# icbi-lab/infercnvpy

Hardware: AMD Instinct MI355X
Metric: cells/sec through tl.infercnv (window=100), input resident in HBM (higher is better)
Workload: dtype f64

## Files before the change

infercnvpy_amd/csrc/icv_api.hip:

```cpp
#include "../../include/infercnv_hip.h"

#include <hip/hip_runtime.h>

#include <algorithm>
#include <atomic>
#include <cmath>
#include <cstdio>
#include <cstdlib>
#include <cstring>
#include <mutex>
#include <new>
#include <string>
#include <system_error>
#include <thread>
#if defined(__x86_64__)
#include <immintrin.h>
#endif
#include <memory>
#include <vector>

#include <rocprim/device/device_radix_sort.hpp>
#include <rocprim/device/device_reduce_by_key.hpp>
#include <rocprim/device/device_scan.hpp>

// ... 1176 lines not shown
        partial_off = 0;
        start_off = up(partial_off + (size_t)n_slabs * nc * 8);
        slab_rec_off = up(start_off + (size_t)n_slabs * nc * 8);
        rec_off = up(slab_rec_off + (size_t)n_slabs * nc * 4);
        count_off = up(rec_off + (size_t)n_blocks * nc * 4);
        stash_off = up(count_off + 256);
        const size_t want = (size_t)n_blocks * nc / 32 + 4096;
        stash_cap = (unsigned)(want < 0x7ffffff0u ? want : 0x7ffffff0u);
        bytes = up(stash_off + (size_t)stash_cap * icv::kBkRows * 4);
    }
};
int blocks_check(const icv_matrix* m, const void* ws) {
    if (!m || !ws) return fail(ICV_ERR_INVALID, "null matrix or workspace");
    if (m->format != ICV_DENSE || m->dtype != ICV_F32)
        return fail(ICV_ERR_UNSUPPORTED, "the block form of the chain takes dense float32 matrices (others: icv_colchain)");
    if (m->n_rows < 0 || m->n_cols < 1 || m->ld < m->n_cols) return fail(ICV_ERR_INVALID, "bad matrix");
    return ICV_OK;
}
}

int icv_colchain_blocks_workspace(int64_t n_rows, int32_t n_cols, int64_t* bytes) {
    if (!bytes || n_rows < 0 || n_cols < 1) return fail(ICV_ERR_INVALID, "bad colchain_blocks_workspace arguments");
    *bytes = (int64_t)BlocksLayout(n_rows, n_cols).bytes;
    return ICV_OK;
}

int icv_colchain_blocks_sums(const icv_matrix* m, void* workspace, double* total, void* stream) {
    int rc = blocks_check(m, workspace);
    if (rc) return rc;
    if (!total) return fail(ICV_ERR_INVALID, "total is required");
    hipStream_t st = static_cast<hipStream_t>(stream);
    const BlocksLayout L(m->n_rows, m->n_cols);
    double* partial = reinterpret_cast<double*>(static_cast<char*>(workspace) + L.partial_off);
    HIP_TRY(hipMemsetAsync(total, 0, (size_t)m->n_cols * sizeof(double), st));
    if (m->n_rows == 0) return ICV_OK;
    dim3 grid((m->n_cols + 255) / 256, (unsigned)L.n_slabs);
    hipLaunchKernelGGL(icv::k_colsum_dense<float>, grid, dim3(256), 0, st, (const float*)m->values, m->n_rows, m->ld,
                       m->n_cols, (const int32_t*)nullptr, 0, icv::kBkSlab, partial);
    hipLaunchKernelGGL(icv::k_colsum_finish, dim3((m->n_cols + 63) / 64), dim3(1024), 0, st, partial, (int)L.n_slabs,
                       m->n_cols, total);
    HIP_TRY(hipGetLastError());
    return ICV_OK;
}

int icv_colchain_blocks_records(const icv_matrix* m, void* workspace, const double* est_start, void* stream) {
    int rc = blocks_check(m, workspace);
    if (rc) return rc;
    if (m->n_rows == 0) return ICV_OK;
    hipStream_t st = static_cast<hipStream_t>(stream);
    const BlocksLayout L(m->n_rows, m->n_cols);
    char* w = static_cast<char*>(workspace);
    const double* partial = reinterpret_cast<const double*>(w + L.partial_off);
    double* slab_start = reinterpret_cast<double*>(w + L.start_off);
    HIP_TRY(hipMemsetAsync(w + L.count_off, 0, 256, st));
    hipLaunchKernelGGL(icv::k_blocks_prefix, dim3((m->n_cols + 255) / 256), dim3(256), 0, st, partial, (int)L.n_slabs,
                       m->n_cols, est_start, slab_start);
    dim3 grid((m->n_cols + 255) / 256, (unsigned)L.n_slabs);
    hipLaunchKernelGGL(icv::k_chain_records, grid, dim3(256), 0, st, (const float*)m->values, m->n_rows, m->ld, m->n_cols,
                       slab_start, reinterpret_cast<uint32_t*>(w + L.rec_off), reinterpret_cast<uint32_t*>(w + L.slab_rec_off),
                       reinterpret_cast<float*>(w + L.stash_off), reinterpret_cast<unsigned*>(w + L.count_off), L.stash_cap);
    HIP_TRY(hipGetLastError());
    return ICV_OK;
}

int icv_colchain_blocks_scan(const icv_matrix* m, void* workspace, float* acc, int32_t col0, int32_t col1,
                             uint64_t* d_replayed, void* stream) {
    int rc = blocks_check(m, workspace);
    if (rc) return rc;
    if (!acc || col0 < 0 || col1 > m->n_cols || col0 > col1) return fail(ICV_ERR_INVALID, "bad colchain_blocks_scan arguments");
    if (m->n_rows == 0 || col1 == col0) return ICV_OK;
    hipStream_t st = static_cast<hipStream_t>(stream);
    const BlocksLayout L(m->n_rows, m->n_cols);
    char* w = static_cast<char*>(workspace);
    const int nc = col1 - col0;
    int64_t grid = ((int64_t)nc + 3) / 4;
    const int64_t cap = (int64_t)current_cu_count() * 8;
    if (grid > cap) grid = cap;
    hipLaunchKernelGGL(icv::k_chain_scan, dim3((unsigned)grid), dim3(256), 0, st,
                       (const float*)m->values + col0, m->n_rows, m->ld, nc, (int64_t)m->n_cols,
                       reinterpret_cast<const uint32_t*>(w + L.rec_off) + col0,
                       reinterpret_cast<const uint32_t*>(w + L.slab_rec_off) + col0,
                       reinterpret_cast<const float*>(w + L.stash_off), acc + col0,
                       reinterpret_cast<unsigned long long*>(d_replayed));
    HIP_TRY(hipGetLastError());
    return ICV_OK;
}

int icv_colchain(const icv_matrix* m, const int32_t* rows, int64_t n_sel, double scale, void* acc, void* stream) {
    if (!m || !acc) return fail(ICV_ERR_INVALID, "bad colchain arguments");
    if (m->dtype != ICV_F32 && m->dtype != ICV_F64) return fail(ICV_ERR_INVALID, "dtype must be ICV_F32 or ICV_F64");
    if (!rows) n_sel = m->n_rows;
    if (n_sel < 0 || n_sel > m->n_rows) return fail(ICV_ERR_INVALID, "icv_colchain: n_sel out of range");
    if (n_sel == 0 || m->n_cols == 0) return ICV_OK;
    hipStream_t st = static_cast<hipStream_t>(stream);
    if (m->format == ICV_CSR)
        return m->dtype == ICV_F32 ? colchain_csr<float>(m, rows, n_sel, scale, (float*)acc, st)
                                   : colchain_csr<double>(m, rows, n_sel, scale, (double*)acc, st);
    if (m->format != ICV_DENSE) return fail(ICV_ERR_INVALID, "format must be dense or csr");
    return m->dtype == ICV_F32 ? colchain_dense<float>(m, rows, n_sel, (float*)acc, st)
                               : colchain_dense<double>(m, rows, n_sel, (double*)acc, st);
}

int icv_colchain_mean(const void* acc, int32_t dtype, int32_t n_cols, int64_t count, void* mean, void* stream) {
    if (!acc || !mean || count < 1 || n_cols < 0) return fail(ICV_ERR_INVALID, "bad colchain_mean arguments");
    hipStream_t st = static_cast<hipStream_t>(stream);
    if (n_cols == 0) return ICV_OK;
    if (dtype == ICV_F32)
        hipLaunchKernelGGL(k_chain_mean<float>, dim3((n_cols + 255) / 256), dim3(256), 0, st, (const float*)acc, n_cols,
                           (float)count, (float*)mean);
    else if (dtype == ICV_F64)
        hipLaunchKernelGGL(k_chain_mean<double>, dim3((n_cols + 255) / 256), dim3(256), 0, st, (const double*)acc,
                           n_cols, (double)count, (double*)mean);
    else
        return fail(ICV_ERR_INVALID, "dtype must be ICV_F32 or ICV_F64");
    HIP_TRY(hipGetLastError());
    return ICV_OK;
}

int icv_colmean_csc(const void* values, int32_t dtype, const int64_t* colptr, const int32_t* row_idx, int32_t n_cols,
                    const int32_t* row_group, int32_t group, double scale, void* mean, void* stream) {
    if (!values || !colptr || !row_idx || !mean || n_cols < 0) return fail(ICV_ERR_INVALID, "bad colmean_csc arguments");
    hipStream_t st = static_cast<hipStream_t>(stream);
    if (n_cols == 0) return ICV_OK;
    if (dtype == ICV_F32)
        hipLaunchKernelGGL(icv::k_colpair_csc<float>, dim3((n_cols + 63) / 64), dim3(64), 0, st, (const float*)values,
                           colptr, row_idx, n_cols, row_group, group, (float)scale, (float*)mean);
    else if (dtype == ICV_F64)
        hipLaunchKernelGGL(icv::k_colpair_csc<double>, dim3((n_cols + 63) / 64), dim3(64), 0, st, (const double*)values,
                           colptr, row_idx, n_cols, row_group, group, scale, (double*)mean);
    else
        return fail(ICV_ERR_INVALID, "dtype must be ICV_F32 or ICV_F64");
    HIP_TRY(hipGetLastError());
    return ICV_OK;
}

int icv_colsum_pairwise(const void* xt, int32_t dtype, int64_t n_rows, int32_t n_cols, int64_t ld, void* sums,
                        void* stream) {
    if (!xt || !sums || n_rows < 0 || n_cols < 0 || ld < n_rows) return fail(ICV_ERR_INVALID, "bad colsum_pairwise arguments");
    hipStream_t st = static_cast<hipStream_t>(stream);
    if (n_cols == 0) return ICV_OK;
    if (dtype == ICV_F32)
        hipLaunchKernelGGL(icv::k_colpair_dense<float>, dim3((n_cols + 63) / 64), dim3(64), 0, st, (const float*)xt,
                           n_rows, n_cols, ld, (float*)sums);
    else if (dtype == ICV_F64)
        hipLaunchKernelGGL(icv::k_colpair_dense<double>, dim3((n_cols + 63) / 64), dim3(64), 0, st, (const double*)xt,
                           n_rows, n_cols, ld, (double*)sums);
    else
        return fail(ICV_ERR_INVALID, "dtype must be ICV_F32 or ICV_F64");
    HIP_TRY(hipGetLastError());
    return ICV_OK;
}

int icv_infercnv_smooth(icv_plan_t pl, const icv_matrix* m, const void* ref_lo, const void* ref_hi,
                        double lfc_clip, int32_t flags, float* out, int64_t ldo, double* cell_median,
                        double* cell_stats, void* stream) {
    int rc = check_matrix(pl, m);
    if (rc) return rc;
    PLAN_BUSY_GUARD(pl);
    if (!cell_median || !cell_stats) return fail(ICV_ERR_INVALID, "cell_median and cell_stats are required");
    if ((rc = ensure_device(pl))) return rc;
    PLAN_ENTER(stream);
    icv::KParams K;
    const icv::Layout* lay;
    if ((rc = fill_params(pl, m, ref_lo, ref_hi, lfc_clip, flags, out, ldo, cell_median, cell_stats, K, lay)))
        return rc;
    return launch_smooth(pl, m, K, *lay, static_cast<hipStream_t>(stream));
}

int icv_chunk_thresholds(const double* cell_stats, int64_t n_rows, int64_t chunksize, int64_t row_phase,
                         int32_t n_windows, double dynamic_threshold, double* thr, void* stream) {
    if (!cell_stats || !thr || chunksize < 1 || row_phase < 0 || row_phase >= chunksize)
        return fail(ICV_ERR_INVALID, "bad chunk threshold arguments");
    if (n_rows < 1) return ICV_OK;
    const int64_t n_chunks = (n_rows + row_phase + chunksize - 1) / chunksize;
    hipLaunchKernelGGL(icv::k_chunk_thr, dim3((unsigned)n_chunks), dim3(256), 0, static_cast<hipStream_t>(stream),
                       cell_stats, n_rows, chunksize, row_phase, n_windows, dynamic_threshold, thr);
    HIP_TRY(hipGetLastError());
    return ICV_OK;
}

int icv_apply_threshold(icv_plan_t pl, const icv_matrix* m, const void* ref_lo, const void* ref_hi,
                        double lfc_clip, int32_t flags, float* out, int64_t ldo, const double* cell_median,
                        const double* thr, int64_t chunksize, int64_t row_phase, void* stream) {
    int rc = check_matrix(pl, m);
    if (rc) return rc;
    PLAN_BUSY_GUARD(pl);
    if (!cell_median || !thr || chunksize < 1) return fail(ICV_ERR_INVALID, "bad apply_threshold arguments");
    if ((rc = ensure_device(pl))) return rc;
    PLAN_ENTER(stream);
    icv::KParams K;
    const icv::Layout* lay;
    if ((rc = fill_params(pl, m, ref_lo, ref_hi, lfc_clip, flags, out, ldo, const_cast<double*>(cell_median),
                          nullptr, K, lay)))
        return rc;
    return launch_apply(m, K, thr, chunksize, row_phase, static_cast<hipStream_t>(stream));
}

}

namespace {
int run_steps(icv_plan_t pl, const icv_matrix* m, const void* ref_lo, const void* ref_hi, double lfc_clip,
              double dynamic_threshold, int64_t chunksize, int64_t row_phase, int32_t flags, float* out, int64_t ldo,
              double* cell_median, double* cell_stats, double* thr, icv_profile* prof, double* win_out, int64_t ldw,
              void* stream) {
    int rc;
    const bool do_thr = !std::isnan(dynamic_threshold);
    hipStream_t st = static_cast<hipStream_t>(stream);
    icv::KParams K;
    const icv::Layout* lay;
    if ((rc = fill_params(pl, m, ref_lo, ref_hi, lfc_clip, flags, out, ldo, cell_median, cell_stats, K, lay)))
        return rc;
    K.win_out = win_out;
    K.win_ld = ldw;
    bool chunk_mode = false;
    int64_t n_chunks = 1, cs_eff = m->n_rows > 0 ? m->n_rows : 1, ph_eff = 0;
    if (do_thr) {
        cs_eff = chunksize;
        ph_eff = row_phase;
        n_chunks = (m->n_rows + row_phase + chunksize - 1) / chunksize;
        if (n_chunks < 1) n_chunks = 1;
    }
    if (!cell_stats && m->n_rows > 0) {
        if (pl->hb_stats_cap < m->n_rows) {
            (void)hipFree(pl->d_hb_stats);
            pl->d_hb_stats = nullptr;
            pl->hb_stats_cap = 0;
            HIP_TRY(hipMalloc((void**)&pl->d_hb_stats, (size_t)m->n_rows * 2 * sizeof(double)));
            pl->hb_stats_cap = m->n_rows;
        }
        K.cell_stats = pl->d_hb_stats;
        const int64_t se_slots = ((int64_t)pl->n_cu * (icv::kLdsLimit / icv::kSeLds)) * icv::NWAVE;
        const int64_t x16_slots = (int64_t)pl->n_cu * icv::XWAVE;
        const int64_t n_part = se_slots > x16_slots ? se_slots : x16_slots;
        if ((x16_applies(pl, m, K, *lay) || stored_entries_kernel(pl, m, K, *lay)) &&
            n_chunks * n_part <= (int64_t)(64 << 20) / 16) {
            chunk_mode = true;
            if (pl->chunk_part_cap < n_chunks * n_part) {
                (void)hipFree(pl->d_chunk_part);
                pl->d_chunk_part = nullptr;
                pl->chunk_part_cap = 0;
                HIP_TRY(hipMalloc((void**)&pl->d_chunk_part, (size_t)(n_chunks * n_part) * 2 * sizeof(double)));
                pl->chunk_part_cap = n_chunks * n_part;
            }
            HIP_TRY(hipMemsetAsync(pl->d_chunk_part, 0, (size_t)(n_chunks * n_part) * 2 * sizeof(double), st));
            HIP_TRY(hipMemsetAsync(pl->d_hb_stats, 0, (size_t)m->n_rows * 2 * sizeof(double), st));
            K.chunk_part = pl->d_chunk_part;
            K.chunksize = cs_eff;
            K.row_phase = ph_eff;
        }
    }
    EventSet evs;
    hipEvent_t* ev = evs.ev;
    const bool deferred = !prof && pl->prof_deferred;
    const bool timed = prof || deferred;
    if (timed) {
        for (int i = 0; i < 4; ++i) HIP_TRY(hipEventCreate(&ev[i]));
        HIP_TRY(hipEventRecord(ev[0], st));
    }
    bool ev1_done = false;
    if ((rc = launch_smooth(pl, m, K, *lay, st, timed ? ev[1] : nullptr, &ev1_done))) return rc;
    if (timed && !ev1_done) HIP_TRY(hipEventRecord(ev[1], st));
    if (do_thr && chunk_mode) {
        int64_t n_slots;
        if (m->format == ICV_CSR) {
            n_slots = se_grid(pl, m->n_rows) * icv::NWAVE;
        } else {
            int64_t gx = pl->n_cu;
            if (gx > m->n_rows) gx = m->n_rows;
            n_slots = gx * icv::XWAVE;
        }
        hipLaunchKernelGGL(icv::k_chunk_thr_part, dim3((unsigned)n_chunks), dim3(256), 0, st, pl->d_chunk_part,
                           (int)n_slots, pl->d_hb_stats, m->n_rows, chunksize, row_phase, pl->p.W,
                           dynamic_threshold, thr);
        HIP_TRY(hipGetLastError());
    } else if (do_thr && m->n_rows > 0) {
        rc = icv_chunk_thresholds(K.cell_stats, m->n_rows, chunksize, row_phase, pl->p.W, dynamic_threshold, thr,
                                  stream);
        if (rc) return rc;
    }
    if (timed) HIP_TRY(hipEventRecord(ev[2], st));
    if (do_thr && !(flags & ICV_FLAG_NO_APPLY) && (rc = launch_apply(m, K, thr, chunksize, row_phase, st))) return rc;
    if (timed) HIP_TRY(hipEventRecord(ev[3], st));
    if (deferred) {
        for (int i = 0; i < 4; ++i) pl->prof_events.push_back(ev[i]);
        evs.keep = true;
    } else if (prof) {
        HIP_TRY(hipEventSynchronize(ev[3]));
        HIP_TRY(hipEventElapsedTime(&prof->smooth_ms, ev[0], ev[1]));
        HIP_TRY(hipEventElapsedTime(&prof->thresholds_ms, ev[1], ev[2]));
        HIP_TRY(hipEventElapsedTime(&prof->apply_ms, ev[2], ev[3]));
        HIP_TRY(hipEventElapsedTime(&prof->total_ms, ev[0], ev[3]));
    }
    return ICV_OK;
}

int gene_from_windows(icv_plan_t pl, const double* win, int64_t ldw, int64_t n, const double* thr, int64_t chunksize,
                      int64_t row_phase, double* gene_out, int64_t ldg, hipStream_t st) {
    const icv::Plan& p = pl->p;
    if (n < 1) return ICV_OK;
    const int W = p.W, n_cov = (int)p.cov_col.size(), R = (int)p.gv_run_j0.size();
    const bool pk_lds = icv::gv_lds_bytes(W, R, pl->gv_mult_bytes, true) * 2 <= (size_t)icv::kLdsLimit;
    const size_t lds = icv::gv_lds_bytes(W, R, pl->gv_mult_bytes, pk_lds);
    if (lds <= (size_t)icv::kLdsLimit && pl->gv_fused_ok && !knobs().no_gene_fused) {
        HIP_TRY(hipFuncSetAttribute(reinterpret_cast<const void*>(icv::k_gene_fused),
                                    hipFuncAttributeMaxDynamicSharedMemorySize, (int)lds));
        int per_cu = (int)((size_t)icv::kLdsLimit / lds);
        if (per_cu > 2048 / icv::kGvThreads) per_cu = 2048 / icv::kGvThreads;
        int64_t grid = (int64_t)pl->n_cu * per_cu;
        if (grid > n) grid = n;
        hipLaunchKernelGGL(icv::k_gene_fused, dim3((unsigned)grid), dim3(icv::kGvThreads), lds, st, win, ldw, n, W,
                           pl->d_gv_pk, pl->d_gv_mult, R, n_cov, pl->d_gv_col16, p.n_cols_all, thr,
                           chunksize > 0 ? chunksize : 1, row_phase, gene_out, ldg, pl->gv_mult_bytes, (int)pk_lds);
        HIP_TRY(hipGetLastError());
        return ICV_OK;
    }
    AsyncBuf b_gv, b_med;
    HIP_TRY(b_gv.alloc((size_t)n * (n_cov > 0 ? n_cov : 1) * sizeof(double), st));
    HIP_TRY(b_med.alloc((size_t)n * sizeof(double), st));
    double *gv = b_gv.as<double>(), *med = b_med.as<double>();
    {
        const int64_t total = n * ldg;
        hipLaunchKernelGGL(icv::k_fill_nan, dim3((unsigned)((total + 255) / 256)), dim3(256), 0, st, gene_out, total);
    }
    if (n_cov > 0) {
        for (int64_t r0 = 0; r0 < n; r0 += 32768) {
            const int64_t nr = (n - r0) < 32768 ? (n - r0) : 32768;
            dim3 grid((n_cov + 255) / 256, (unsigned)nr);
            hipLaunchKernelGGL(icv::k_gene_means, grid, dim3(256), 0, st, win + r0 * ldw, nr, (int)ldw, pl->d_cov_j0,
                               pl->d_cov_cnt, n_cov, gv + r0 * n_cov);
        }
        hipLaunchKernelGGL(icv::k_row_median, dim3((unsigned)n), dim3(256), 0, st, gv, n, n_cov, med);
        for (int64_t r0 = 0; r0 < n; r0 += 32768) {
            const int64_t nr = (n - r0) < 32768 ? (n - r0) : 32768;
            dim3 grid((n_cov + 255) / 256, (unsigned)nr);
            hipLaunchKernelGGL(icv::k_gene_finish, grid, dim3(256), 0, st, gv + r0 * n_cov, med + r0, thr,
                               chunksize > 0 ? chunksize : 1, row_phase + r0, pl->d_cov_col, n_cov, gene_out + r0 * ldg,
                               ldg);
        }
    }
    HIP_TRY(hipGetLastError());
    return ICV_OK;
}
}

extern "C" {

int icv_infercnv_run(icv_plan_t pl, const icv_matrix* m, const void* ref_lo, const void* ref_hi, double lfc_clip,
                     double dynamic_threshold, int64_t chunksize, int64_t row_phase, int32_t flags, float* out,
                     int64_t ldo, double* cell_median, double* cell_stats, double* thr, icv_profile* prof,
                     void* stream) {
    return icv_infercnv_run_windows(pl, m, ref_lo, ref_hi, lfc_clip, dynamic_threshold, chunksize, row_phase, flags, out,
                                    ldo, cell_median, cell_stats, thr, prof, nullptr, 0, stream);
}

int icv_infercnv_run_windows(icv_plan_t pl, const icv_matrix* m, const void* ref_lo, const void* ref_hi,
                             double lfc_clip, double dynamic_threshold, int64_t chunksize, int64_t row_phase,
                             int32_t flags, float* out, int64_t ldo, double* cell_median, double* cell_stats,
                             double* thr, icv_profile* prof, double* win_out, int64_t ldw, void* stream) {
    int rc = check_matrix(pl, m);
    if (rc) return rc;
    PLAN_BUSY_GUARD(pl);
    const bool do_thr = !std::isnan(dynamic_threshold);
    if (m->n_rows == 0) return ICV_OK;
    if (!cell_median) return fail(ICV_ERR_INVALID, "cell_median is required");
    if (do_thr && (!thr || chunksize < 1 || row_phase < 0 || row_phase >= chunksize))
        return fail(ICV_ERR_INVALID, "thr buffer / chunksize / row_phase invalid");
    if (win_out && ldw < pl->p.W) return fail(ICV_ERR_INVALID, "ldw < n_windows");
    if ((rc = ensure_device(pl))) return rc;
    PLAN_ENTER(stream);
    return run_steps(pl, m, ref_lo, ref_hi, lfc_clip, dynamic_threshold, chunksize, row_phase, flags, out, ldo,
                     cell_median, cell_stats, thr, prof, win_out, ldw, stream);
}

int icv_gene_values_from_windows(icv_plan_t pl, const double* win, int64_t ldw, int64_t n_rows, const double* thr,
                                 int64_t chunksize, int64_t row_phase, double* gene_out, int64_t ldg, void* stream) {
    if (!pl) return fail(ICV_ERR_INVALID, "null plan");
    PLAN_BUSY_GUARD(pl);
    if (n_rows < 0 || (n_rows > 0 && (!win || !gene_out)) || ldw < pl->p.W || ldg < pl->p.n_cols_all)
        return fail(ICV_ERR_INVALID, "bad gene_values_from_windows arguments (null buffer, ldw < n_windows or ldg < n_cols)");
    if (thr && (chunksize < 1 || row_phase < 0 || row_phase >= chunksize))
        return fail(ICV_ERR_INVALID, "chunksize / row_phase invalid");
    int rc;
    if ((rc = ensure_device(pl))) return rc;
    PLAN_ENTER(stream);
    return gene_from_windows(pl, win, ldw, n_rows, thr, chunksize, row_phase, gene_out, ldg,
                             static_cast<hipStream_t>(stream));
}

int icv_profile_begin(icv_plan_t pl) {
    if (!pl) return fail(ICV_ERR_INVALID, "null plan");
    for (auto& e : pl->prof_events) (void)hipEventDestroy(e);
    pl->prof_events.clear();
    pl->prof_deferred = true;
    return ICV_OK;
}

int icv_profile_collect(icv_plan_t pl, icv_profile* out, int32_t max_records, int32_t* n_records) {
    if (!pl || !n_records || (max_records > 0 && !out)) return fail(ICV_ERR_INVALID, "bad profile_collect arguments");
    const int n = (int)(pl->prof_events.size() / 4);
    int k = 0;
    for (int i = 0; i < n; ++i) {
        hipEvent_t* ev = pl->prof_events.data() + 4 * i;
        if (k < max_records) {
            HIP_TRY(hipEventSynchronize(ev[3]));
            HIP_TRY(hipEventElapsedTime(&out[k].smooth_ms, ev[0], ev[1]));
            HIP_TRY(hipEventElapsedTime(&out[k].thresholds_ms, ev[1], ev[2]));
            HIP_TRY(hipEventElapsedTime(&out[k].apply_ms, ev[2], ev[3]));
            HIP_TRY(hipEventElapsedTime(&out[k].total_ms, ev[0], ev[3]));
            ++k;
        }
    }
    for (auto& e : pl->prof_events) (void)hipEventDestroy(e);
    pl->prof_events.clear();
    pl->prof_deferred = false;
    *n_records = k;
    return ICV_OK;
}

int icv_gene_values(icv_plan_t pl, const icv_matrix* m, const void* ref_lo, const void* ref_hi, double lfc_clip,
                    int32_t flags, const double* thr, int64_t chunksize, int64_t row_phase, double* gene_out,
                    int64_t ldg, void* stream) {
    int rc = check_matrix(pl, m);
    if (rc) return rc;
    PLAN_BUSY_GUARD(pl);
    if (!gene_out || ldg < m->n_cols) return fail(ICV_ERR_INVALID, "gene_out is null or ldg < n_cols");
    if (thr && (chunksize < 1 || row_phase < 0 || row_phase >= chunksize))
        return fail(ICV_ERR_INVALID, "chunksize / row_phase invalid");
    if ((rc = ensure_device(pl))) return rc;
    PLAN_ENTER(stream);
    const int64_t n = m->n_rows;
    if (n < 1) return ICV_OK;
    hipStream_t st = static_cast<hipStream_t>(stream);
    const int W = pl->p.W;
    AsyncBuf b_out32, b_win, b_cmed;
    HIP_TRY(b_out32.alloc((size_t)n * W * sizeof(float), st));
    HIP_TRY(b_win.alloc((size_t)n * W * sizeof(double), st));
    HIP_TRY(b_cmed.alloc((size_t)n * sizeof(double), st));
    if ((rc = run_steps(pl, m, ref_lo, ref_hi, lfc_clip, std::nan(""), 1, 0, flags, b_out32.as<float>(), W,
                        b_cmed.as<double>(), nullptr, nullptr, nullptr, b_win.as<double>(), W, stream)))
        return rc;
    return gene_from_windows(pl, b_win.as<double>(), W, n, thr, chunksize, row_phase, gene_out, ldg, st);
}

int icv_threshold_mask(icv_plan_t pl, const icv_matrix* m, const void* ref_lo, const void* ref_hi, double lfc_clip,
                       int32_t flags, const float* out, int64_t ldo, const double* cell_median, const double* thr,
                       int64_t chunksize, int64_t row_phase, uint64_t* mask, int64_t* row_nnz, void* stream) {
    int rc = check_matrix(pl, m);
    if (rc) return rc;
    PLAN_BUSY_GUARD(pl);
    if (!cell_median || !mask || !row_nnz || (thr && (chunksize < 1 || row_phase < 0 || row_phase >= chunksize)))
        return fail(ICV_ERR_INVALID, "bad threshold_mask arguments");
    if ((rc = ensure_device(pl))) return rc;
    PLAN_ENTER(stream);
    icv::KParams K;
    const icv::Layout* lay;
    if ((rc = fill_params(pl, m, ref_lo, ref_hi, lfc_clip, flags, const_cast<float*>(out), ldo,
                          const_cast<double*>(cell_median), nullptr, K, lay)))
        return rc;
    if (K.n_rows < 1) return ICV_OK;
    hipStream_t st = static_cast<hipStream_t>(stream);
    const int n_words = (pl->p.W + 63) / 64;
    const int64_t cs = thr ? chunksize : 1;
    auto* mk = reinterpret_cast<unsigned long long*>(mask);
    const icv::PackRing pr(pl->p.W);
    const bool ring = !knobs().no_mask_ring && pr.ok && (ldo & 3) == 0 && (reinterpret_cast<uintptr_t>(out) & 15) == 0 &&
                      (reinterpret_cast<uintptr_t>(mask) & 7) == 0;
    if (ring) {
        const int lds = pr.lds_bytes();
        const int64_t rounds = (K.n_rows + icv::kPmRows - 1) / icv::kPmRows;
        const unsigned gx = (unsigned)(rounds < pl->n_cu ? rounds : pl->n_cu);
        AsyncBuf ties;
        if (thr) HIP_TRY(ties.alloc((size_t)K.n_rows * icv::kPmPerRow * sizeof(unsigned long long), st));
        HIP_TRY(hipFuncSetAttribute(reinterpret_cast<const void*>(icv::k_thr_mask_ring),
                                    hipFuncAttributeMaxDynamicSharedMemorySize, icv::kPmLds));
        hipLaunchKernelGGL(icv::k_thr_mask_ring, dim3(gx), dim3(icv::kPmThreads), lds, st, K, thr, cs, row_phase, mk, n_words,
                           row_nnz, pl->d_tie_n, ties.as<unsigned long long>());
        if (thr) {
            dim3 tg(128), tb(256);
            const auto* tl = ties.as<unsigned long long>();
            if (m->dtype == ICV_F32) {
                if (m->format == ICV_DENSE)
                    hipLaunchKernelGGL((icv::k_thr_mask_ties<float, false>), tg, tb, 0, st, K, thr, cs, row_phase, mk, n_words, row_nnz, pl->d_tie_n, tl);
                else
                    hipLaunchKernelGGL((icv::k_thr_mask_ties<float, true>), tg, tb, 0, st, K, thr, cs, row_phase, mk, n_words, row_nnz, pl->d_tie_n, tl);
            } else {
                if (m->format == ICV_DENSE)
                    hipLaunchKernelGGL((icv::k_thr_mask_ties<double, false>), tg, tb, 0, st, K, thr, cs, row_phase, mk, n_words, row_nnz, pl->d_tie_n, tl);
                else
                    hipLaunchKernelGGL((icv::k_thr_mask_ties<double, true>), tg, tb, 0, st, K, thr, cs, row_phase, mk, n_words, row_nnz, pl->d_tie_n, tl);
            }
        }
        HIP_TRY(hipGetLastError());
        return ICV_OK;
    }
    dim3 grid((unsigned)K.n_rows), block(256);
    if (m->dtype == ICV_F32) {
        if (m->format == ICV_DENSE)
            hipLaunchKernelGGL((icv::k_thr_mask<float, false>), grid, block, 0, st, K, thr, cs, row_phase, mk, n_words, row_nnz);
        else
            hipLaunchKernelGGL((icv::k_thr_mask<float, true>), grid, block, 0, st, K, thr, cs, row_phase, mk, n_words, row_nnz);
    } else {
        if (m->format == ICV_DENSE)
            hipLaunchKernelGGL((icv::k_thr_mask<double, false>), grid, block, 0, st, K, thr, cs, row_phase, mk, n_words, row_nnz);
        else
            hipLaunchKernelGGL((icv::k_thr_mask<double, true>), grid, block, 0, st, K, thr, cs, row_phase, mk, n_words, row_nnz);
    }
    HIP_TRY(hipGetLastError());
    return ICV_OK;
}

int icv_threshold_pack(icv_plan_t pl, const icv_matrix* m, const void* ref_lo, const void* ref_hi, double lfc_clip,
                       int32_t flags, const float* out, int64_t ldo, const double* cell_median, const double* thr,
                       int64_t chunksize, int64_t row_phase, int64_t* indptr, int32_t* indices, double* data,
                       int64_t capacity, void* stream) {
    int rc = check_matrix(pl, m);
    if (rc) return rc;
    PLAN_BUSY_GUARD(pl);
    if (!cell_median || !indptr || !indices || !data || capacity < 0 ||
        (thr && (chunksize < 1 || row_phase < 0 || row_phase >= chunksize)))
        return fail(ICV_ERR_INVALID, "bad threshold_pack arguments");
    if (pl->p.W > 320 * 64) return fail(ICV_ERR_UNSUPPORTED, "icv_threshold_pack: more than 20480 windows");
    const int n_words = (pl->p.W + 63) / 64;
    int rpw = icv::kPackWords / n_words;
    rpw = rpw < 1 ? 1 : (rpw > icv::kPackMaxRows ? icv::kPackMaxRows : rpw);
    if ((rc = ensure_device(pl))) return rc;
    PLAN_ENTER(stream);
    icv::KParams K;
    const icv::Layout* lay;
    if ((rc = fill_params(pl, m, ref_lo, ref_hi, lfc_clip, flags, const_cast<float*>(out), ldo,
                          const_cast<double*>(cell_median), nullptr, K, lay)))
        return rc;
    hipStream_t st = static_cast<hipStream_t>(stream);
    if (K.n_rows < 1) {
        HIP_TRY(hipMemsetAsync(indptr, 0, sizeof(int64_t), st));
        return ICV_OK;
    }
    if (K.n_rows > 0xffffffffll) return fail(ICV_ERR_UNSUPPORTED, "icv_threshold_pack: more than 2^32 rows per call");
    const int64_t n_tickets = (K.n_rows + rpw - 1) / rpw, n_groups = (n_tickets + 63) / 64;
    AsyncBuf ws;
    HIP_TRY(ws.alloc((size_t)(n_tickets + 2 * n_groups + 1) * sizeof(unsigned long long), st));
    HIP_TRY(hipMemsetAsync(ws.p, 0, (size_t)(n_tickets + 2 * n_groups + 1) * sizeof(unsigned long long), st));
    auto* status = ws.as<unsigned long long>();
    auto* gstat = status + n_tickets;
    auto* gacc = gstat + n_groups;
    auto* ticket = reinterpret_cast<unsigned int*>(gacc + n_groups);
    const int64_t cs = thr ? chunksize : 1;
    dim3 grid((unsigned)n_tickets), block(256);
#define ICV_PACK(TT, CC) \
    hipLaunchKernelGGL((icv::k_thr_pack<TT, CC>), grid, block, 0, st, K, thr, cs, row_phase, rpw, ticket, status, gstat, gacc, indptr, indices, data, capacity)
    if (m->dtype == ICV_F32) {
        if (m->format == ICV_DENSE) ICV_PACK(float, false);
        else ICV_PACK(float, true);
    } else {
        if (m->format == ICV_DENSE) ICV_PACK(double, false);
        else ICV_PACK(double, true);
    }
#undef ICV_PACK
    HIP_TRY(hipGetLastError());
    return ICV_OK;
}

int icv_pack_geometry(int32_t n_windows, icv_pack_info* info) {
    if (!info || n_windows < 1) return fail(ICV_ERR_INVALID, "bad pack_geometry arguments");
    const icv::PackRing pr(n_windows);
    const icv::FillRing fr(n_windows);
    info->rows_per_round = icv::kPmRows;
    info->mask_streamed = pr.ok ? 1 : 0;
    info->mask_ring_slots = pr.ok ? pr.n_slots : 0;
    info->mask_lds_bytes = pr.ok ? pr.lds_bytes() : 0;
    info->mask_loads_in_flight = pr.ok ? (pr.n_slots - 1) * pr.per_loader : 0;
    info->fill_streamed = fr.ok ? 1 : 0;
    info->fill_ring_slots = fr.ok ? fr.n_slots : 0;
    info->fill_lds_bytes = fr.ok ? fr.lds_bytes() : 0;
    info->fill_loads_in_flight = fr.ok ? (fr.n_slots - 1) * (fr.per_loader + fr.n_extra) : 0;
    info->fill_stage_entries = fr.ok ? fr.cap : 0;
    return ICV_OK;
}

int icv_row_offsets(const int64_t* row_nnz, int64_t n_rows, int64_t* indptr, void* stream) {
    if ((!row_nnz && n_rows > 0) || !indptr || n_rows < 0) return fail(ICV_ERR_INVALID, "bad row_offsets arguments");
    hipStream_t st = static_cast<hipStream_t>(stream);
    const unsigned nb = (unsigned)((n_rows + icv::kScanBlock - 1) / icv::kScanBlock);
    AsyncBuf sums;
    HIP_TRY(sums.alloc((size_t)(nb ? nb : 1) * sizeof(int64_t), st));
    if (nb > 1) hipLaunchKernelGGL(icv::k_row_block_sums, dim3(nb), dim3(1024), 0, st, row_nnz, n_rows, sums.as<int64_t>());
    hipLaunchKernelGGL(icv::k_row_offsets, dim3(nb ? nb : 1), dim3(1024), 0, st, row_nnz, n_rows, sums.as<int64_t>(), indptr);
    HIP_TRY(hipGetLastError());
    return ICV_OK;
}

int icv_csr_fill_masked(const float* x, int64_t n_rows, int32_t n_cols, int64_t ld, const uint64_t* mask,
                        const int64_t* indptr, int32_t* indices, double* data, void* stream) {
    if (!x || !mask || !indptr || !indices || !data || n_cols < 0 || ld < n_cols)
        return fail(ICV_ERR_INVALID, "bad csr_fill_masked arguments");
    if (n_rows < 1) return ICV_OK;
    hipStream_t st = static_cast<hipStream_t>(stream);
    const icv::FillRing fr(n_cols);
    if (!knobs().no_fill_ring && fr.ok && (ld & 3) == 0 && (reinterpret_cast<uintptr_t>(x) & 15) == 0 &&
        (reinterpret_cast<uintptr_t>(mask) & 7) == 0) {
        const int n_cu = current_cu_count();
        const int64_t rounds = (n_rows + icv::kPmRows - 1) / icv::kPmRows;
        const unsigned gx = (unsigned)(rounds < n_cu ? rounds : n_cu);
        HIP_TRY(hipFuncSetAttribute(reinterpret_cast<const void*>(icv::k_csr_fill_ring),
                                    hipFuncAttributeMaxDynamicSharedMemorySize, icv::kPmLds));
        hipLaunchKernelGGL(icv::k_csr_fill_ring, dim3(gx), dim3(icv::kPmThreads), fr.lds_bytes(), st, x, n_rows, n_cols, ld,
                           reinterpret_cast<const unsigned long long*>(mask), indptr, indices, data);
        HIP_TRY(hipGetLastError());
        return ICV_OK;
    }
    hipLaunchKernelGGL(icv::k_csr_fill_masked, dim3((unsigned)((n_rows + 3) / 4)), dim3(256), 0, st, x, n_rows, n_cols, ld,
                       reinterpret_cast<const unsigned long long*>(mask), (n_cols + 63) / 64, indptr, indices, data);
    HIP_TRY(hipGetLastError());
    return ICV_OK;
// ... 2322 lines not shown
```

infercnvpy_amd/csrc/icv_kernel_gene.hpp:

```cpp
#pragma once
#include "icv_kernels.hpp"

namespace icv {

constexpr int kGvThreads = 512;
constexpr int kGvWaves = kGvThreads / 64;
constexpr int kGvBins = 4 * kGvThreads;
constexpr int kGvCand = 64;

struct GvScratch {
    unsigned hist[kGvBins];
    double red[2][kGvWaves];
    double cand_v[kGvCand];
    int cand_w[kGvCand];
    int wsum[kGvWaves];
    int ncand, anynan, sel_bin, sel_below;
    double v1, v2;
    int found2, pad_;
};

__host__ __device__ inline size_t gv_lds_bytes(int W, int R, int mult_bytes = 2, bool pk_lds = false) {
    size_t w = (size_t)W * 8;
    if (w < sizeof(GvScratch)) w = sizeof(GvScratch);
    w = (w + 15) / 16 * 16;
    return w + ((size_t)R + 2) * 8 + ((size_t)R * mult_bytes + 15) / 16 * 16 + (pk_lds ? (size_t)R * 4 : 0);
}

__device__ __forceinline__ double gv_numpy_sum(const double* a, int n) {
    if (n < 8) {
        double r = 0.0;
        for (int i = 0; i < n; ++i) r += a[i];
        return r;
    }
    if (n <= 128) {
        double r[8];
#pragma unroll
        for (int k = 0; k < 8; ++k) r[k] = a[k];
        int i = 8;
        for (; i + 8 <= n; i += 8) {
#pragma unroll
            for (int k = 0; k < 8; ++k) r[k] += a[i + k];
        }
        double res = ((r[0] + r[1]) + (r[2] + r[3])) + ((r[4] + r[5]) + (r[6] + r[7]));
        for (; i < n; ++i) res += a[i];
        return res;
    }
    return __builtin_nan("");
}

__global__ void __launch_bounds__(kGvThreads) k_gene_fused(
    const double* __restrict__ win, int64_t ldw, int64_t n_rows, int W, const uint32_t* __restrict__ run_pk,
    const int32_t* __restrict__ run_mult, int R, int n_cov, const uint16_t* __restrict__ col_run16, int n_cols,
    const double* __restrict__ thr, int64_t chunksize, int64_t row_phase, double* __restrict__ out, int64_t ldg,
    int mult_bytes, int pk_lds) {
    extern __shared__ __attribute__((aligned(16))) unsigned char gsm[];
    size_t woff = (size_t)W * 8;
    if (woff < sizeof(GvScratch)) woff = sizeof(GvScratch);
    woff = (woff + 15) / 16 * 16;
    double* lwin = reinterpret_cast<double*>(gsm);
    GvScratch* sc = reinterpret_cast<GvScratch*>(gsm);
    double* val = reinterpret_cast<double*>(gsm + woff);
    const size_t vbytes = ((size_t)R + 2) * 8;
    unsigned short* mult16 = reinterpret_cast<unsigned short*>(gsm + woff + vbytes);
    unsigned char* mult8 = reinterpret_cast<unsigned char*>(mult16);
    uint32_t* lpk = reinterpret_cast<uint32_t*>(gsm + woff + vbytes + ((size_t)R * mult_bytes + 15) / 16 * 16);
    const bool m8 = mult_bytes == 1;
    const auto mult_of = [&](int r) { return m8 ? (int)mult8[r] : (int)mult16[r]; };
    const int t = threadIdx.x, lane = t & 63, wave = t >> 6;
    const int k1 = (n_cov - 1) / 2, k2 = n_cov / 2;
    for (int i = t; i < R; i += kGvThreads) {
        if (m8) mult8[i] = (unsigned char)run_mult[i];
        else mult16[i] = (unsigned short)run_mult[i];
        if (pk_lds) lpk[i] = run_pk[i];
    }
    if (t == 0) val[R] = __builtin_nan("");
    const bool vec2 = (ldg % 2 == 0) && ((reinterpret_cast<uintptr_t>(out) & 15) == 0);
    const bool win16 = (ldw % 2 == 0) && ((reinterpret_cast<uintptr_t>(win) & 15) == 0);
    const double nan = __builtin_nan("");
    constexpr int UW = 4;
    constexpr int UR = 4;
    constexpr int UC = 20;
    constexpr int PW = 2;
    typedef double f64x2_t __attribute__((ext_vector_type(2)));
    f64x2_t pre[PW];
    const int n2w = W / 2;
    const auto prefetch = [&](int64_t cell_) {
        const double* wr_ = win + cell_ * ldw;
#pragma unroll
        for (int u = 0; u < PW; ++u)
            if (t + u * kGvThreads < n2w) pre[u] = *reinterpret_cast<const f64x2_t*>(wr_ + 2 * (t + u * kGvThreads));
    };
    if (win16 && (int64_t)blockIdx.x < n_rows) prefetch(blockIdx.x);
    for (int64_t cell = blockIdx.x; cell < n_rows; cell += gridDim.x) {
        __syncthreads();
        const double* wr = win + cell * ldw;
        if (win16) {
#pragma unroll
            for (int u = 0; u < PW; ++u)
                if (t + u * kGvThreads < n2w) *reinterpret_cast<f64x2_t*>(lwin + 2 * (t + u * kGvThreads)) = pre[u];
            const int n2 = W / 2;
            for (int j0 = t + PW * kGvThreads; j0 < n2; j0 += UW * kGvThreads) {
                f64x2_t q[UW];
#pragma unroll
                for (int u = 0; u < UW; ++u)
                    if (j0 + u * kGvThreads < n2) q[u] = *reinterpret_cast<const f64x2_t*>(wr + 2 * (j0 + u * kGvThreads));
#pragma unroll
                for (int u = 0; u < UW; ++u)
                    if (j0 + u * kGvThreads < n2) *reinterpret_cast<f64x2_t*>(lwin + 2 * (j0 + u * kGvThreads)) = q[u];
            }
            if ((W & 1) && t == 0) lwin[W - 1] = wr[W - 1];
        } else {
            for (int j = t; j < W; j += kGvThreads) lwin[j] = wr[j];
        }
        __syncthreads();
        int nanl = 0;
        double mn = __builtin_inf(), mx = -__builtin_inf();
        for (int r0 = t; r0 < R; r0 += UR * kGvThreads) {
            uint32_t pk[UR];
#pragma unroll
            for (int u = 0; u < UR; ++u)
                pk[u] = r0 + u * kGvThreads < R ? (pk_lds ? lpk[r0 + u * kGvThreads] : run_pk[r0 + u * kGvThreads]) : 0u;
#pragma unroll
            for (int u = 0; u < UR; ++u) {
                const int r = r0 + u * kGvThreads;
                if (r < R) {
                    const int cnt = (int)(pk[u] >> 16);
                    const double v = gv_numpy_sum(lwin + (pk[u] & 0xffffu), cnt) / (double)cnt;
                    val[r] = v;
                    nanl |= (v != v);
                    mn = v < mn ? v : mn;
                    mx = v > mx ? v : mx;
                }
            }
        }
        mn = wave_min_dpp(mn);
        mx = wave_max_dpp(mx);
        __syncthreads();
        if (t == 0) {
            sc->anynan = 0;
            sc->found2 = 0;
        }
        if (lane == 0) {
            sc->red[0][wave] = mn;
            sc->red[1][wave] = mx;
        }
        __syncthreads();
        if (nanl) sc->anynan = 1;
        double lo = sc->red[0][0], hi = sc->red[1][0];
#pragma unroll
        for (int i = 1; i < kGvWaves; ++i) {
            lo = sc->red[0][i] < lo ? sc->red[0][i] : lo;
            hi = sc->red[1][i] > hi ? sc->red[1][i] : hi;
        }
        __syncthreads();
        const bool anynan = sc->anynan != 0;
        double v1 = lo, v2 = lo;
#if defined(ICV_DEV_EXPERIMENTS) && defined(GV_EXP_NOMEDIAN)
        if (false) {
#else
        if (!anynan && R > 0) {
#endif
            int below = 0;
            bool need2 = k2 != k1;
            for (int level = 0; level < 64; ++level) {
                if (!(hi > lo)) {
                    v1 = lo;
                    int w = 0;
                    for (int r = t; r < R; r += kGvThreads) w += (val[r] == lo) ? mult_of(r) : 0;
                    w = wave_sum_i(w);
                    if (lane == 0) sc->wsum[wave] = w;
                    __syncthreads();
                    int wt = 0;
#pragma unroll
                    for (int i = 0; i < kGvWaves; ++i) wt += sc->wsum[i];
                    if (need2 && k2 - below < wt) {
                        v2 = lo;
                        need2 = false;
                    }
                    break;
                }
                for (int i = t; i < kGvBins; i += kGvThreads) sc->hist[i] = 0u;
                if (t == 0) sc->ncand = 0;
                __syncthreads();
                const double scale = (double)kGvBins / (hi - lo);
                for (int r = t; r < R; r += kGvThreads) {
                    const double v = val[r];
                    if (v >= lo && v <= hi) {
                        int b = (int)((v - lo) * scale);
                        b = b > kGvBins - 1 ? kGvBins - 1 : b;
                        atomicAdd(&sc->hist[b], (unsigned)mult_of(r));
                    }
                }
                __syncthreads();
                const int kk = k1 - below;
                const uint4 h = reinterpret_cast<const uint4*>(sc->hist)[t];
                const int c = (int)((h.x + h.y) + (h.z + h.w));
                const int incl = wave_scan_dpp(c);
                if (lane == 63) sc->wsum[wave] = incl;
                __syncthreads();
                int wbase = 0;
#pragma unroll
                for (int i = 0; i < kGvWaves; ++i) wbase += i < wave ? sc->wsum[i] : 0;
                const int excl = wbase + incl - c;
                if (kk >= excl && kk < excl + c) {
                    int run = excl, d = 3;
                    if (kk < run + (int)h.x) d = 0;
                    else if (kk < run + (int)(h.x + h.y)) { d = 1; run += (int)h.x; }
                    else if (kk < run + (int)(h.x + h.y + h.z)) { d = 2; run += (int)(h.x + h.y); }
                    else run += (int)(h.x + h.y + h.z);
                    sc->sel_bin = 4 * t + d;
                    sc->sel_below = run;
                }
                __syncthreads();
                const int sb = sc->sel_bin;
                below += sc->sel_below;
                double bmn = __builtin_inf(), bmx = -__builtin_inf();
                for (int r = t; r < R; r += kGvThreads) {
                    const double v = val[r];
                    if (v >= lo && v <= hi) {
                        int b = (int)((v - lo) * scale);
                        b = b > kGvBins - 1 ? kGvBins - 1 : b;
                        if (b == sb) {
                            const int idx = atomicAdd(&sc->ncand, 1);
                            if (idx < kGvCand) {
                                sc->cand_v[idx] = v;
                                sc->cand_w[idx] = mult_of(r);
                            }
                            bmn = v < bmn ? v : bmn;
                            bmx = v > bmx ? v : bmx;
                        }
                    }
                }
                bmn = wave_min_dpp(bmn);
                bmx = wave_max_dpp(bmx);
                if (lane == 0) {
                    sc->red[0][wave] = bmn;
                    sc->red[1][wave] = bmx;
                }
                __syncthreads();
                const int nc = sc->ncand;
                if (nc <= kGvCand) {
                    if (wave == 0) {
                        const double mine = lane < nc ? sc->cand_v[lane] : __builtin_inf();
                        int wl = 0, we = 0;
                        for (int q = 0; q < nc; ++q) {
                            const double o = sc->cand_v[q];
                            const int w = sc->cand_w[q];
                            wl += o < mine ? w : 0;
                            we += o == mine ? w : 0;
                        }
                        const int ka = k1 - below, kb = k2 - below;
                        if (lane < nc && ka >= wl && ka < wl + we) sc->v1 = mine;
                        if (lane < nc && kb >= wl && kb < wl + we) {
                            sc->v2 = mine;
                            sc->found2 = 1;
                        }
                    }
                    __syncthreads();
                    v1 = sc->v1;
                    if (need2 && sc->found2) {
                        v2 = sc->v2;
                        need2 = false;
                    }
                    break;
                }
                lo = sc->red[0][0];
                hi = sc->red[1][0];
#pragma unroll
                for (int i = 1; i < kGvWaves; ++i) {
                    lo = sc->red[0][i] < lo ? sc->red[0][i] : lo;
                    hi = sc->red[1][i] > hi ? sc->red[1][i] : hi;
                }
                __syncthreads();
            }
            if (need2) {
                double m2 = __builtin_inf();
                for (int r = t; r < R; r += kGvThreads) {
                    const double v = val[r];
                    if (v > v1 && v < m2) m2 = v;
                }
                m2 = wave_min_dpp(m2);
                __syncthreads();
                if (lane == 0) sc->red[0][wave] = m2;
                __syncthreads();
                v2 = sc->red[0][0];
#pragma unroll
                for (int i = 1; i < kGvWaves; ++i) v2 = sc->red[0][i] < v2 ? sc->red[0][i] : v2;
            } else if (k2 == k1) {
                v2 = v1;
            }
        }
        const double med = anynan ? nan : ((k1 == k2) ? v1 : (v1 + v2) / 2.0);
        const bool has_thr = thr != nullptr;
        const double th = has_thr ? thr[(cell + row_phase) / chunksize] : 0.0;
        double* orow = out + cell * ldg;
        for (int r = t; r < R; r += kGvThreads) {
            double a = val[r] - med;
            if (has_thr && fabs(a) < th) a = 0.0;
            val[r] = a;
        }
        __syncthreads();
        const auto value_of = [&](unsigned rx) { return val[rx]; };
        if (vec2) {
            const int n2 = (n_cols + 1) / 2;
            const uint32_t* cr2 = reinterpret_cast<const uint32_t*>(col_run16);
            for (int g0 = t; g0 < n2; g0 += UC * kGvThreads) {
                uint32_t rr[UC];
#pragma unroll
                for (int u = 0; u < UC; ++u) rr[u] = g0 + u * kGvThreads < n2 ? cr2[g0 + u * kGvThreads] : 0u;
                if (g0 + UC * kGvThreads >= n2 && win16 && cell + gridDim.x < n_rows) prefetch(cell + gridDim.x);
#pragma unroll
                for (int u = 0; u < UC; ++u) {
                    const int c = 2 * (g0 + u * kGvThreads);
                    if (c >= n_cols) continue;
                    const double a = value_of(rr[u] & 0xffffu), b = value_of(rr[u] >> 16);
                    if (c + 2 <= n_cols) {
                        const f64x2_t q = {a, b};
#if defined(ICV_DEV_EXPERIMENTS) && defined(GV_EXP_PLAIN)
                        *reinterpret_cast<f64x2_t*>(orow + c) = q;
#elif defined(ICV_DEV_EXPERIMENTS) && defined(GV_EXP_NOSTORE)
                        if (a == 1.2345e300) *reinterpret_cast<f64x2_t*>(orow + c) = q;
#else
                        __builtin_nontemporal_store(q, reinterpret_cast<f64x2_t*>(orow + c));
#endif
                    } else {
                        orow[c] = a;
                    }
                }
            }
        } else {
            if (win16 && cell + gridDim.x < n_rows) prefetch(cell + gridDim.x);
            for (int c = t; c < n_cols; c += kGvThreads) orow[c] = value_of((unsigned)col_run16[c]);
        }
    }
}

}
```

Baseline: 32.86 million.

## Keep column-run table in registers and overlap prior row's stores with run means

Adds a templated resident variant of the fused gene kernel. It loads the column-to-run index table into registers once per block and defers each row's output scatter into the next row's run-mean loop, using buffer stores interleaved with the window summation. A final tail store handles the last row. This removes the per-row reload of the index table from memory and hides store latency behind compute. In exchange it raises register pressure, changes the launch-bounds occupancy hint, and keeps run means in registers until after the reduction.

```diff
diff --git a/infercnvpy_amd/csrc/icv_api.hip b/infercnvpy_amd/csrc/icv_api.hip
--- a/infercnvpy_amd/csrc/icv_api.hip
+++ b/infercnvpy_amd/csrc/icv_api.hip
@@ -1502,13 +1502,15 @@
     const bool pk_lds = icv::gv_lds_bytes(W, R, pl->gv_mult_bytes, true) * 2 <= (size_t)icv::kLdsLimit;
     const size_t lds = icv::gv_lds_bytes(W, R, pl->gv_mult_bytes, pk_lds);
     if (lds <= (size_t)icv::kLdsLimit && pl->gv_fused_ok && !knobs().no_gene_fused) {
-        HIP_TRY(hipFuncSetAttribute(reinterpret_cast<const void*>(icv::k_gene_fused),
-                                    hipFuncAttributeMaxDynamicSharedMemorySize, (int)lds));
+        auto* const kern = icv::gv_table_resident(p.n_cols_all, R, pk_lds, ldg, gene_out) ? icv::k_gene_fused<true>
+                                                                                          : icv::k_gene_fused<false>;
+        HIP_TRY(hipFuncSetAttribute(reinterpret_cast<const void*>(kern), hipFuncAttributeMaxDynamicSharedMemorySize,
+                                    (int)lds));
         int per_cu = (int)((size_t)icv::kLdsLimit / lds);
         if (per_cu > 2048 / icv::kGvThreads) per_cu = 2048 / icv::kGvThreads;
         int64_t grid = (int64_t)pl->n_cu * per_cu;
         if (grid > n) grid = n;
-        hipLaunchKernelGGL(icv::k_gene_fused, dim3((unsigned)grid), dim3(icv::kGvThreads), lds, st, win, ldw, n, W,
+        hipLaunchKernelGGL(kern, dim3((unsigned)grid), dim3(icv::kGvThreads), lds, st, win, ldw, n, W,
                            pl->d_gv_pk, pl->d_gv_mult, R, n_cov, pl->d_gv_col16, p.n_cols_all, thr,
                            chunksize > 0 ? chunksize : 1, row_phase, gene_out, ldg, pl->gv_mult_bytes, (int)pk_lds);
         HIP_TRY(hipGetLastError());
diff --git a/infercnvpy_amd/csrc/icv_kernel_gene.hpp b/infercnvpy_amd/csrc/icv_kernel_gene.hpp
--- a/infercnvpy_amd/csrc/icv_kernel_gene.hpp
+++ b/infercnvpy_amd/csrc/icv_kernel_gene.hpp
@@ -48,7 +48,21 @@
     return __builtin_nan("");
 }
 
-__global__ void __launch_bounds__(kGvThreads) k_gene_fused(
+#if defined(ICV_DEV_EXPERIMENTS) && defined(GV_EXP_PLAIN)
+constexpr int kGvStoreAux = 0;
+#else
+constexpr int kGvStoreAux = 2;
+#endif
+constexpr int kGvResWords = 20;
+constexpr int kGvResRuns = 8;
+
+__host__ __device__ inline bool gv_table_resident(int n_cols, int R, bool pk_lds, int64_t ldg, const void* out) {
+    return (ldg % 2 == 0) && ((reinterpret_cast<uintptr_t>(out) & 15) == 0) &&
+           (n_cols + 1) / 2 <= kGvResWords * kGvThreads && R <= kGvResRuns * kGvThreads && pk_lds;
+}
+
+template <bool RES>
+__global__ void __launch_bounds__(kGvThreads, RES ? 4 : 2) k_gene_fused(
     const double* __restrict__ win, int64_t ldw, int64_t n_rows, int W, const uint32_t* __restrict__ run_pk,
     const int32_t* __restrict__ run_mult, int R, int n_cov, const uint16_t* __restrict__ col_run16, int n_cols,
     const double* __restrict__ thr, int64_t chunksize, int64_t row_phase, double* __restrict__ out, int64_t ldg,
@@ -79,7 +93,7 @@
     const double nan = __builtin_nan("");
     constexpr int UW = 4;
     constexpr int UR = 4;
-    constexpr int UC = 20;
+    constexpr int UC = kGvResWords;
     constexpr int PW = 2;
     typedef double f64x2_t __attribute__((ext_vector_type(2)));
     f64x2_t pre[PW];
@@ -91,6 +105,27 @@
             if (t + u * kGvThreads < n2w) pre[u] = *reinterpret_cast<const f64x2_t*>(wr_ + 2 * (t + u * kGvThreads));
     };
     if (win16 && (int64_t)blockIdx.x < n_rows) prefetch(blockIdx.x);
+    uint32_t rres[RES ? UC : 1];
+    unsigned last_run = (unsigned)R;
+    if constexpr (RES) {
+        const int n2 = n_cols / 2;
+        const uint32_t* cr2 = reinterpret_cast<const uint32_t*>(col_run16);
+#pragma unroll
+        for (int u = 0; u < UC; ++u)
+            rres[u] = t + u * kGvThreads < n2 ? cr2[t + u * kGvThreads] : (uint32_t)R * 0x10001u;
+        if (n_cols & 1) last_run = col_run16[n_cols - 1];
+#pragma unroll
+        for (int u = 0; u < PW; ++u) asm volatile("" : "+v"(pre[u]));
+    }
+    const auto store_pair = [&](const __amdgpu_buffer_rsrc_t o_rs, int t_, int u) {
+        const uint32_t w = rres[RES ? u : 0];
+        const f64x2_t q = {val[w & 0xffffu], val[w >> 16]};
+#if defined(ICV_DEV_EXPERIMENTS) && defined(GV_EXP_NOSTORE)
+        if (q.x == 1.2345e300)
+#endif
+        __builtin_amdgcn_raw_buffer_store_b128(__builtin_bit_cast(u32x4, q), o_rs, (unsigned)t_ * 16u,
+                                               u * kGvThreads * 16, kGvStoreAux);
+    };
     for (int64_t cell = blockIdx.x; cell < n_rows; cell += gridDim.x) {
         __syncthreads();
         const double* wr = win + cell * ldw;
@@ -115,22 +150,50 @@
         __syncthreads();
         int nanl = 0;
         double mn = __builtin_inf(), mx = -__builtin_inf();
-        for (int r0 = t; r0 < R; r0 += UR * kGvThreads) {
-            uint32_t pk[UR];
-#pragma unroll
-            for (int u = 0; u < UR; ++u)
-                pk[u] = r0 + u * kGvThreads < R ? (pk_lds ? lpk[r0 + u * kGvThreads] : run_pk[r0 + u * kGvThreads]) : 0u;
-#pragma unroll
-            for (int u = 0; u < UR; ++u) {
-                const int r = r0 + u * kGvThreads;
+        double rv[RES ? kGvResRuns : 1];
+        if constexpr (RES) {
+            const bool has_prev = cell != (int64_t)blockIdx.x;
+            double* prow = out + (has_prev ? cell - (int64_t)gridDim.x : cell) * ldg;
+            if (has_prev && (n_cols & 1) && t == 0) prow[n_cols - 1] = val[last_run];
+            const __amdgpu_buffer_rsrc_t o_rs = make_rsrc(prow, has_prev ? (unsigned)(n_cols >> 1) * 16u : 0u);
+            int tl = t;
+            asm volatile("" : "+v"(tl));
+#pragma unroll
+            for (int u = 0; u < UC; ++u) asm volatile("" : "+v"(rres[u]));
+#pragma unroll
+            for (int i = 0; i < kGvResRuns; ++i) {
+                const int r = tl + i * kGvThreads;
+                rv[i] = 0.0;
                 if (r < R) {
-                    const int cnt = (int)(pk[u] >> 16);
-                    const double v = gv_numpy_sum(lwin + (pk[u] & 0xffffu), cnt) / (double)cnt;
-                    val[r] = v;
+                    const uint32_t pk = lpk[r];
+                    const int cnt = (int)(pk >> 16);
+                    const double v = gv_numpy_sum(lwin + (pk & 0xffffu), cnt) / (double)cnt;
+                    rv[i] = v;
                     nanl |= (v != v);
                     mn = v < mn ? v : mn;
                     mx = v > mx ? v : mx;
                 }
+#pragma unroll
+                for (int u = i * UC / kGvResRuns; u < (i + 1) * UC / kGvResRuns; ++u) store_pair(o_rs, tl, u);
+            }
+        } else {
+            for (int r0 = t; r0 < R; r0 += UR * kGvThreads) {
+                uint32_t pk[UR];
+#pragma unroll
+                for (int u = 0; u < UR; ++u)
+                    pk[u] = r0 + u * kGvThreads < R ? (pk_lds ? lpk[r0 + u * kGvThreads] : run_pk[r0 + u * kGvThreads]) : 0u;
+#pragma unroll
+                for (int u = 0; u < UR; ++u) {
+                    const int r = r0 + u * kGvThreads;
+                    if (r < R) {
+                        const int cnt = (int)(pk[u] >> 16);
+                        const double v = gv_numpy_sum(lwin + (pk[u] & 0xffffu), cnt) / (double)cnt;
+                        val[r] = v;
+                        nanl |= (v != v);
+                        mn = v < mn ? v : mn;
+                        mx = v > mx ? v : mx;
+                    }
+                }
             }
         }
         mn = wave_min_dpp(mn);
@@ -143,6 +206,12 @@
         if (lane == 0) {
             sc->red[0][wave] = mn;
             sc->red[1][wave] = mx;
+        }
+        if constexpr (RES) {
+            if (win16 && cell + gridDim.x < n_rows) prefetch(cell + gridDim.x);
+#pragma unroll
+            for (int i = 0; i < kGvResRuns; ++i)
+                if (t + i * kGvThreads < R) val[t + i * kGvThreads] = rv[i];
         }
         __syncthreads();
         if (nanl) sc->anynan = 1;
@@ -301,7 +370,8 @@
         }
         __syncthreads();
         const auto value_of = [&](unsigned rx) { return val[rx]; };
-        if (vec2) {
+        if constexpr (RES) {
+        } else if (vec2) {
             const int n2 = (n_cols + 1) / 2;
             const uint32_t* cr2 = reinterpret_cast<const uint32_t*>(col_run16);
             for (int g0 = t; g0 < n2; g0 += UC * kGvThreads) {
@@ -333,6 +403,16 @@
             for (int c = t; c < n_cols; c += kGvThreads) orow[c] = value_of((unsigned)col_run16[c]);
         }
     }
+    if constexpr (RES) {
+        if ((int64_t)blockIdx.x < n_rows) {
+            const int64_t cell = blockIdx.x + (n_rows - 1 - blockIdx.x) / gridDim.x * gridDim.x;
+            double* prow = out + cell * ldg;
+            if ((n_cols & 1) && t == 0) prow[n_cols - 1] = val[last_run];
+            const __amdgpu_buffer_rsrc_t o_rs = make_rsrc(prow, (unsigned)(n_cols >> 1) * 16u);
+#pragma unroll
+            for (int u = 0; u < UC; ++u) store_pair(o_rs, t, u);
+        }
+    }
 }
 
 }
```

Result: slower. 31.93 million (-2.8%).
